# omerbt/TokenFlow

Hardware: NVIDIA H100
Metric: frames/sec for 40-frame 512x512 SD1.5 50-step edit (higher is better)
Workload: dtype fp16

## Files before the change

include/tokenflow_b200.h:

```cpp
#ifndef TOKENFLOW_B200_H_
#define TOKENFLOW_B200_H_

#include <stdint.h>

#ifdef __cplusplus
extern "C" {
#endif

typedef void* tf_stream_t;

#define TF_MAX_FRAMES 64
#define TF_MAX_ATTN_SAMPLES 160

int tf_version(void);
const char* tf_last_error(void);
int64_t tf_launch_count(void);

int tf_unit_rows(const void* x, int x_is_f32, int64_t rows, int dim, int64_t x_row_stride, void* out_f16,
                 tf_stream_t stream);

int tf_layernorm_unit_rows(const void* x_f16, int64_t rows, int dim, int64_t x_row_stride, const float* gamma,
                           const float* beta, float eps, void* out_f16, tf_stream_t stream);

int tf_layernorm_rows(const void* x_f16, int64_t rows, int dim, int64_t x_row_stride, const float* gamma,
// ... 15 lines not shown
                         const int32_t* q_slab, const int32_t* k_slab0, const int32_t* v_slab0,
                         const int32_t* n_kv, int S, int heads, int d, float scale, int q_row0, int q_nrows,
                         void* out, tf_stream_t stream);

int tf_cfg_ddim(const void* eps_uncond, const void* eps_cond, const void* x, const float* coef, float guidance,
                int64_t n, void* out, tf_stream_t stream);

int tf_ddim(const void* eps, const void* x, const float* coef, int64_t n, void* out, tf_stream_t stream);


int tf_cfg_ddim_v(const void* v_uncond, const void* v_cond, const void* x, const float* coef, float guidance,
                  int64_t n, void* out, tf_stream_t stream);

int tf_ddim_v(const void* v, const void* x, const float* coef, int64_t n, void* out, tf_stream_t stream);


int64_t tf_group_norm_nhwc_workspace(int64_t n, int64_t hw, int c, int groups);
int tf_group_norm_nhwc(const void* x, const void* bias, int64_t bias_stride, const void* gamma, const void* beta,
                       int64_t n, int64_t hw, int c, int groups, float eps, int silu, void* workspace,
                       int64_t workspace_bytes, void* out, tf_stream_t stream);

int tf_geglu(const void* xh, const void* gate, int64_t n, void* out, tf_stream_t stream);


int tf_frames_to_nhwc(const void* frames_u8, int64_t n_px, void* out_f16, tf_stream_t stream);

int tf_nhwc_to_frames(const void* x_f16, int64_t n_px, void* frames_u8, tf_stream_t stream);

int tf_resize_taps(int in, int out);
int tf_resize_coeffs(int in, int out, int32_t* bounds, int32_t* coeffs);
int tf_resize_u8(const void* in, int64_t n, int h_in, int w_in, int h, int w, const int32_t* h_bounds,
                 const int32_t* h_coeffs, int h_taps, const int32_t* v_bounds, const int32_t* v_coeffs, int v_taps,
                 void* tmp, void* out, tf_stream_t stream);

int64_t tf_canny_workspace(int64_t n, int h, int w);
int tf_canny_u8(const void* frames, int64_t n, int h, int w, double low, double high, void* workspace,
                int64_t workspace_bytes, void* edges_u8, void* cond_f16, tf_stream_t stream);

#define TF_COMM_ID_BYTES 128
typedef void* tf_comm_t;
int tf_comm_nccl_version(void);
int tf_comm_unique_id(void* id_out);
int tf_comm_init(const void* id, int nranks, int rank, tf_comm_t* comm_out);
int tf_allgather(tf_comm_t comm, const void* send, void* recv, int64_t bytes_per_rank, tf_stream_t stream);
int tf_comm_destroy(tf_comm_t comm);

// ... 5 lines not shown
```

tokenflow_b200/_build.py:

```python
from __future__ import annotations

import hashlib
import os
import shutil
import subprocess
import sys
from pathlib import Path

PKG_DIR = Path(__file__).resolve().parent
CSRC = PKG_DIR / "csrc"
LIB_PATH = PKG_DIR / "libtokenflow_b200.so"
STAMP = PKG_DIR / ".libtokenflow_b200.stamp"

SOURCES = ["tf_capi.cu", "tf_unit_rows.cu", "tf_propagate.cu", "tf_nn_field.cu", "tf_ext_attn.cu", "tf_cfg_ddim.cu",
           "tf_comm.cu", "tf_body.cu", "tf_pixels.cu", "tf_resize.cu",
           "tf_canny.cu"]
HEADERS = ["tf_common.cuh", "tf_kernels.h", "tf_wgmma.cuh", "../../include/tokenflow_b200.h"]

NVCC_FLAGS = [
    "-gencode", "arch=compute_90a,code=sm_90a",
    "-O3", "-std=c++17", "-lineinfo",
    "-Xcompiler", "-fPIC",
    "-Xcompiler", "-ffp-contract=off",
    "-Xptxas", "-v",
    "--expt-relaxed-constexpr",
    "-cudart", "static",
]


def _nvcc() -> str:
    for cand in (os.environ.get("NVCC"), shutil.which("nvcc"), "/usr/local/cuda/bin/nvcc"):
        if cand and os.path.exists(cand):
            return cand
    raise RuntimeError("nvcc not found (set NVCC=/path/to/nvcc)")


def _digest() -> str:
    h = hashlib.sha256()
    for name in SOURCES + HEADERS:
        h.update((CSRC / name).read_bytes())
# ... 43 lines not shown
```

tokenflow_b200/csrc/tf_body.cu:

```cuda
#include "tf_common.cuh"
#include "tf_kernels.h"

namespace tf {
namespace {

constexpr int kGnMaxThreads = 512;
static_assert(kGnMaxChannels / 8 <= kGnMaxThreads, "one row of 8-channel columns must fit in a CTA");
constexpr int kGnStatsChunkBytes = 64 << 10;
constexpr int kGnApplyChunkBytes = 128 << 10;
constexpr int kGnUnroll = 4;

struct GnLayout {
  int cols, rows, threads;
  long long stats_px, apply_px;
  int stats_chunks, apply_chunks;
};

GnLayout gn_layout(long long hw, int c) {
  GnLayout L;
  L.cols = c / 8;
  L.rows = kGnMaxThreads / L.cols > 0 ? kGnMaxThreads / L.cols : 1;
  L.threads = (L.cols * L.rows + 31) / 32 * 32;
  auto chunk = [&](int bytes) {
    long long px = bytes / (2LL * c);
// ... 191 lines not shown
      if (q < p_end) {
        float v[8];
        unpack8(raw[u], v);
        uint4 w;
        __half2* h = reinterpret_cast<__half2*>(&w);
#pragma unroll
        for (int e = 0; e < 4; ++e) {
          float y[2];
#pragma unroll
          for (int k = 0; k < 2; ++k) {
            const int i = 2 * e + k;
            const float xv = kBias ? round_h(v[i] + bv[i]) : v[i];
            y[k] = round_h(fmaf(a[i], xv, b[i]));
            if (kSilu) y[k] = y[k] / (1.0f + expf(-y[k]));
          }
          h[e] = __floats2half2_rn(y[0], y[1]);
        }
        *reinterpret_cast<uint4*>(on + q * C + c0) = w;
      }
    }
  }
}

__device__ __forceinline__ float gelu_erf(float v) {
  constexpr float kAlpha = 0.70710678118654752440f;
  return v * 0.5f * (1.0f + erff(v * kAlpha));
}

__device__ __forceinline__ float geglu1(float xv, float gv) { return xv * round_h(gelu_erf(gv)); }

__global__ void __launch_bounds__(256)
geglu_kernel(const __half* __restrict__ xh, const __half* __restrict__ gate, long long n_vec, long long n,
             __half* __restrict__ out) {
  const long long stride = (long long)gridDim.x * blockDim.x;
  for (long long i = (long long)blockIdx.x * blockDim.x + threadIdx.x; i < n_vec; i += stride) {
    float xv[8], gv[8];
    unpack8(reinterpret_cast<const uint4*>(xh)[i], xv);
    unpack8(reinterpret_cast<const uint4*>(gate)[i], gv);
    uint4 w;
    __half2* h = reinterpret_cast<__half2*>(&w);
#pragma unroll
    for (int e = 0; e < 4; ++e) h[e] = __floats2half2_rn(geglu1(xv[2 * e], gv[2 * e]), geglu1(xv[2 * e + 1], gv[2 * e + 1]));
    reinterpret_cast<uint4*>(out)[i] = w;
  }
  if (blockIdx.x == 0 && threadIdx.x == 0) {
    for (long long j = n_vec * 8; j < n; ++j)
      out[j] = __float2half_rn(geglu1(__half2float(xh[j]), __half2float(gate[j])));
  }
}

}

long long group_norm_nhwc_workspace(long long n, long long hw, int c, int groups) {
  if (n <= 0 || hw <= 0 || c <= 0 || (c & 7) || groups <= 0 || c % groups) return 0;
  return n * groups * (long long)gn_layout(hw, c).stats_chunks * (long long)sizeof(double2);
}

namespace {

template <int kCpg>
int launch_gn(const GnLayout& L, const __half* xp, const __half* bp, long long bias_stride, const __half* gp,
              const __half* btp, long long n, long long hw, int c, int groups, float eps, int silu, double2* ws,
              __half* op, cudaStream_t stream, const char* stats_what, const char* apply_what) {
  const int cpg = c / groups;
  const size_t stats_smem = (size_t)L.threads * 2 * sizeof(double2);
  const size_t apply_smem = (2 * (size_t)c + 2 * (size_t)groups) * sizeof(float);
  for (long long n0 = 0; n0 < n; n0 += 65535) {
    const unsigned ny = (unsigned)(n - n0 < 65535 ? n - n0 : 65535);
    const long long off = n0 * hw * c;
    const __half* bn = bp ? bp + n0 * bias_stride : nullptr;
// ... 60 lines not shown
```

tokenflow_b200/csrc/tf_capi.cu:

```cuda
#include <algorithm>
#include <atomic>
#include <cmath>
#include <cstdarg>
#include <cstdio>
#include <cstring>
#include <initializer_list>
#include <vector>

#include "../../include/tokenflow_b200.h"
#include "tf_common.cuh"
#include "tf_kernels.h"

namespace tf {

static thread_local char g_err[512] = "";
static std::atomic<long long> g_launches{0};

void set_last_error(const char* fmt, ...) {
  va_list ap;
  va_start(ap, fmt);
  vsnprintf(g_err, sizeof(g_err), fmt, ap);
  va_end(ap);
}

// ... 335 lines not shown
  if (!canny_sizes_ok(n, h, w, "tf_canny_u8")) return TF_ERR_INVALID_ARGUMENT;
  if (!(low == low) || !(high == high)) {
    set_last_error("tf_canny_u8: NaN threshold");
    return TF_ERR_INVALID_ARGUMENT;
  }
  if (low > high) std::swap(low, high);
  const double lo = std::floor(low), hi = std::floor(high);
  const int ilo = (int)std::min(std::max(lo, -1.0), 2040.0), ihi = (int)std::min(std::max(hi, -1.0), 2040.0);
  if (n == 0) return TF_OK;
  const long long need = canny_workspace(n, h, w);
  if (workspace_bytes < need) {
    set_last_error("tf_canny_u8: workspace of %lld bytes, %lld needed", (long long)workspace_bytes, need);
    return TF_ERR_INVALID_ARGUMENT;
  }
  const bool cond_ok = !(reinterpret_cast<uintptr_t>(cond_f16) & 1u);
  if (int e = check_pointers("tf_canny_u8", {workspace}, {}, frames && (edges_u8 || cond_f16) && cond_ok)) return e;
  return launched(
      launch_canny(frames, n, h, w, ilo, ihi, workspace, edges_u8, cond_f16, static_cast<cudaStream_t>(stream)), 5);
}

int tf_geglu(const void* xh, const void* gate, int64_t n, void* out, tf_stream_t stream) {
  return elementwise("tf_geglu", n, INT64_MAX, {xh, gate, out}, true,
                     [&] { return launch_geglu(xh, gate, n, out, static_cast<cudaStream_t>(stream)); });
}

int tf_nn_field(const void* x_unit, const void* piv_unit, const int32_t* kf_a, const int32_t* kf_b, int F, int S,
                int dim, int K, int32_t* idx_a, int32_t* idx_b, tf_stream_t stream) {
  if (F < 0 || S < 0 || dim <= 0 || (dim & 7) || K <= 0) {
    set_last_error("tf_nn_field: bad shape F=%d S=%d dim=%d K=%d", F, S, dim, K);
    return TF_ERR_INVALID_ARGUMENT;
  }
  std::vector<FrameChunk> chunks;
  bool need_b;
  if (int e = frame_chunks(chunks, need_b, kf_a, kf_b, nullptr, F, K, "tf_nn_field")) return e;
  if (F == 0 || S == 0) return TF_OK;
  if (int e = check_pointers("tf_nn_field", {x_unit, piv_unit}, {}, idx_a && (!need_b || idx_b))) return e;
  const __half* xu = static_cast<const __half*>(x_unit);
  for (const FrameChunk& c : chunks) {
    const long long off = (long long)c.f0 * S;
    if (int e = launched(launch_nn_field(xu + off * dim, piv_unit, c.tab, c.n, S, dim, K, idx_a + off,
                                         idx_b ? idx_b + off : nullptr, static_cast<cudaStream_t>(stream))))
      return e;
  }
  return TF_OK;
}

// ... 144 lines not shown
```

tokenflow_b200/csrc/tf_common.cuh:

```cuda
#pragma once

#include <cuda.h>
#include <cuda_fp16.h>
#include <cuda_runtime.h>
#include <stdint.h>
#include <stdio.h>

namespace tf {

void set_last_error(const char* fmt, ...);
int  check_cuda(cudaError_t e, const char* what);

enum Status : int {
  TF_OK = 0,
  TF_ERR_INVALID_ARGUMENT = 1,
  TF_ERR_CUDA = 2,
  TF_ERR_UNSUPPORTED = 3,
  TF_ERR_DRIVER = 4,
};

CUresult encode_tiled(CUtensorMap* map, CUtensorMapDataType dtype, uint32_t rank, const void* base,
                      const uint64_t* dims, const uint64_t* strides_bytes ,
                      const uint32_t* box, CUtensorMapSwizzle swizzle);

// ... 29 lines not shown
      : "memory");
  return ok != 0;
}
__device__ __forceinline__ uint64_t global_timer_ns() {
  uint64_t t;
  asm volatile("mov.u64 %0, %%globaltimer;" : "=l"(t));
  return t;
}
__device__ __forceinline__ void mbar_wait(uint64_t* bar, uint32_t parity) {
  uint32_t spins = 0;
  uint64_t t0 = 0;
  while (!mbar_try_wait(bar, parity)) {
    if ((++spins & 2047u) == 0) {
      const uint64_t now = global_timer_ns();
      if (t0 == 0) t0 = now;
      if (now - t0 > 2000000000ull) __trap();
    }
  }
}

__device__ __forceinline__ void tma_prefetch_desc(const CUtensorMap* m) {
  asm volatile("prefetch.tensormap [%0];" ::"l"(reinterpret_cast<uint64_t>(m)) : "memory");
}
__device__ __forceinline__ void tma_load_3d(void* smem_dst, const CUtensorMap* m, uint64_t* bar, int c0,
                                            int c1, int c2) {
  asm volatile(
      "cp.async.bulk.tensor.3d.shared::cluster.global.tile.mbarrier::complete_tx::bytes"
      " [%0], [%1, {%3, %4, %5}], [%2];"
      ::"r"(smem_u32(smem_dst)), "l"(reinterpret_cast<uint64_t>(m)), "r"(smem_u32(bar)), "r"(c0), "r"(c1),
      "r"(c2)
      : "memory");
}
__device__ __forceinline__ void tma_load_4d(void* smem_dst, const CUtensorMap* m, uint64_t* bar, int c0,
                                            int c1, int c2, int c3) {
  asm volatile(
      "cp.async.bulk.tensor.4d.shared::cluster.global.tile.mbarrier::complete_tx::bytes"
      " [%0], [%1, {%3, %4, %5, %6}], [%2];"
      ::"r"(smem_u32(smem_dst)), "l"(reinterpret_cast<uint64_t>(m)), "r"(smem_u32(bar)), "r"(c0), "r"(c1),
      "r"(c2), "r"(c3)
      : "memory");
}

__device__ __forceinline__ uint64_t wgmma_desc(uint32_t smem_addr, uint32_t lbo_bytes, uint32_t sbo_bytes) {
  uint64_t d = 0;
  d |= static_cast<uint64_t>((smem_addr & 0x3FFFFu) >> 4);
  d |= static_cast<uint64_t>((lbo_bytes >> 4) & 0x3FFFu) << 16;
  d |= static_cast<uint64_t>((sbo_bytes >> 4) & 0x3FFFu) << 32;
  d |= static_cast<uint64_t>(1) << 62;
  return d;
}
__device__ __forceinline__ void wgmma_fence() { asm volatile("wgmma.fence.sync.aligned;" ::: "memory"); }
__device__ __forceinline__ void wgmma_commit() { asm volatile("wgmma.commit_group.sync.aligned;" ::: "memory"); }
template <int kPending>
__device__ __forceinline__ void wgmma_wait() {
  asm volatile("wgmma.wait_group.sync.aligned %0;" ::"n"(kPending) : "memory");
}
template <int N>
__device__ __forceinline__ void reg_fence(float (&r)[N]) {
#pragma unroll
  for (int i = 0; i < N; ++i) asm volatile("" : "+f"(r[i])::"memory");
}

__device__ __forceinline__ uint32_t pack_f16x2_rn(float lo, float hi) {
  uint32_t r;
  asm("cvt.rn.f16x2.f32 %0, %1, %2;" : "=r"(r) : "f"(hi), "f"(lo));
  return r;
}
__device__ __forceinline__ float fast_exp2(float x) {
  float y;
  asm("ex2.approx.ftz.f32 %0, %1;" : "=f"(y) : "f"(x));
  return y;
}
#endif

}
```

tokenflow_b200/csrc/tf_kernels.h:

```cpp
#pragma once

#include <cuda_runtime.h>
#include <stdint.h>

namespace tf {

constexpr int kMaxFrames = 64;
struct FrameTable {
  int32_t kf_a[kMaxFrames];
  int32_t kf_b[kMaxFrames];
  float w[kMaxFrames];
};

int launch_unit_rows(const void* x, int x_is_f32, long long rows, int dim, long long row_stride, void* out_f16,
                     cudaStream_t stream);

int launch_layernorm_unit_rows(const void* x_f16, long long rows, int dim, long long row_stride, const float* gamma,
                               const float* beta, float eps, void* out_f16, cudaStream_t stream);

int launch_layernorm_rows(const void* x_f16, long long rows, int dim, long long row_stride, const float* gamma,
                          const float* beta, float eps, void* y_out, long long y_row_stride, void* unit_out,
                          long long unit_row_stride, long long unit_rows, cudaStream_t stream);

int launch_cfg_ddim(const void* eps_uncond, const void* eps_cond, const void* x, const float* coef_dev, float guidance,
                    long long n, void* out, cudaStream_t stream);
int launch_ddim(const void* eps, const void* x, const float* coef_dev, long long n, void* out, cudaStream_t stream);
int launch_cfg_ddim_v(const void* v_uncond, const void* v_cond, const void* x, const float* coef_dev, float guidance,
                      long long n, void* out, cudaStream_t stream);
int launch_ddim_v(const void* v, const void* x, const float* coef_dev, long long n, void* out, cudaStream_t stream);

constexpr int kGnMaxChannels = 4096;
long long group_norm_nhwc_workspace(long long n, long long hw, int c, int groups);
int launch_group_norm_nhwc(const void* x, const void* bias, long long bias_stride, const void* gamma, const void* beta,
                           long long n, long long hw, int c, int groups, float eps, int silu, void* workspace,
                           void* out, cudaStream_t stream);
int launch_geglu(const void* xh, const void* gate, long long n, void* out, cudaStream_t stream);

int launch_frames_to_nhwc(const void* frames, long long n, void* out, cudaStream_t stream);
int launch_nhwc_to_frames(const void* x, long long n, void* frames, cudaStream_t stream);

int resize_taps(int in, int out);
void resize_coeffs(int in, int out, int32_t* bounds, int32_t* coeffs);
int launch_resize_h(const void* in, long long n_rows, int w_in, int w, const int32_t* bounds, const int32_t* coeffs,
                    int taps, void* out, cudaStream_t stream);
int launch_resize_v(const void* in, long long n, int h_in, int h, int w, const int32_t* bounds, const int32_t* coeffs,
                    int taps, void* out, cudaStream_t stream);

long long canny_workspace(long long n, int h, int w);
int launch_canny(const void* frames, long long n, int h, int w, int low, int high, void* workspace, void* edges,
                 void* cond, cudaStream_t stream);

int launch_propagate(const void* A, const int32_t* idx_a, const int32_t* idx_b, const FrameTable& tab, int F,
                     int S, int dim, int K, const void* residual, void* out, int out_is_f32, long long F_total,
                     cudaStream_t stream);

int launch_nn_field(const void* x_unit, const void* piv_unit, const FrameTable& tab, int F, int S, int dim,
                    int K, int32_t* idx_a, int32_t* idx_b, cudaStream_t stream);

struct AttnSample {
// ... 35 lines not shown
```

tokenflow_b200/csrc/tf_wgmma.cuh:

```cuda
#pragma once

#include <stdint.h>

namespace tf {

template <int N> __device__ __forceinline__ void wgmma_ss(float (&d)[N / 2], uint64_t a, uint64_t b, uint32_t acc);
template <int N> __device__ __forceinline__ void wgmma_rs(float (&d)[N / 2], const uint32_t (&a)[4], uint64_t b, uint32_t acc);

template <>
__device__ __forceinline__ void wgmma_ss<64>(float (&d)[32], uint64_t a, uint64_t b, uint32_t acc) {
  asm volatile(
      "{\n\t.reg .pred p;\n\t"
      "setp.ne.b32 p, %34, 0;\n\t"
      "wgmma.mma_async.sync.aligned.m64n64k16.f32.f16.f16 "
      "{%0, %1, %2, %3, %4, %5, %6, %7, %8, %9, %10, %11, %12, %13, %14, %15, %16, %17, %18, %19, %20, %21, %22, %23, %24, %25, %26, %27, %28, %29, %30, %31}, "
      "%32, %33, p, 1, 1, 0, 0;\n\t}\n"
      : "+f"(d[0]), "+f"(d[1]), "+f"(d[2]), "+f"(d[3]), "+f"(d[4]), "+f"(d[5]), "+f"(d[6]), "+f"(d[7]),
        "+f"(d[8]), "+f"(d[9]), "+f"(d[10]), "+f"(d[11]), "+f"(d[12]), "+f"(d[13]), "+f"(d[14]), "+f"(d[15]),
        "+f"(d[16]), "+f"(d[17]), "+f"(d[18]), "+f"(d[19]), "+f"(d[20]), "+f"(d[21]), "+f"(d[22]), "+f"(d[23]),
        "+f"(d[24]), "+f"(d[25]), "+f"(d[26]), "+f"(d[27]), "+f"(d[28]), "+f"(d[29]), "+f"(d[30]), "+f"(d[31])
      : "l"(a), "l"(b), "r"(acc));
}

template <>
__device__ __forceinline__ void wgmma_ss<128>(float (&d)[64], uint64_t a, uint64_t b, uint32_t acc) {
  asm volatile(
      "{\n\t.reg .pred p;\n\t"
      "setp.ne.b32 p, %66, 0;\n\t"
      "wgmma.mma_async.sync.aligned.m64n128k16.f32.f16.f16 "
      "{%0, %1, %2, %3, %4, %5, %6, %7, %8, %9, %10, %11, %12, %13, %14, %15, %16, %17, %18, %19, %20, %21, %22, %23, %24, %25, %26, %27, %28, %29, %30, %31, %32, %33, %34, %35, %36, %37, %38, %39, %40, %41, %42, %43, %44, %45, %46, %47, %48, %49, %50, %51, %52, %53, %54, %55, %56, %57, %58, %59, %60, %61, %62, %63}, "
// ... 199 lines not shown
template <>
__device__ __forceinline__ void wgmma_rs<192>(float (&d)[96], const uint32_t (&a)[4], uint64_t b, uint32_t acc) {
  asm volatile(
      "{\n\t.reg .pred p;\n\t"
      "setp.ne.b32 p, %101, 0;\n\t"
      "wgmma.mma_async.sync.aligned.m64n192k16.f32.f16.f16 "
      "{%0, %1, %2, %3, %4, %5, %6, %7, %8, %9, %10, %11, %12, %13, %14, %15, %16, %17, %18, %19, %20, %21, %22, %23, %24, %25, %26, %27, %28, %29, %30, %31, %32, %33, %34, %35, %36, %37, %38, %39, %40, %41, %42, %43, %44, %45, %46, %47, %48, %49, %50, %51, %52, %53, %54, %55, %56, %57, %58, %59, %60, %61, %62, %63, %64, %65, %66, %67, %68, %69, %70, %71, %72, %73, %74, %75, %76, %77, %78, %79, %80, %81, %82, %83, %84, %85, %86, %87, %88, %89, %90, %91, %92, %93, %94, %95}, "
      "{%96, %97, %98, %99}, %100, p, 1, 1, 1;\n\t}\n"
      : "+f"(d[0]), "+f"(d[1]), "+f"(d[2]), "+f"(d[3]), "+f"(d[4]), "+f"(d[5]), "+f"(d[6]), "+f"(d[7]),
        "+f"(d[8]), "+f"(d[9]), "+f"(d[10]), "+f"(d[11]), "+f"(d[12]), "+f"(d[13]), "+f"(d[14]), "+f"(d[15]),
        "+f"(d[16]), "+f"(d[17]), "+f"(d[18]), "+f"(d[19]), "+f"(d[20]), "+f"(d[21]), "+f"(d[22]), "+f"(d[23]),
        "+f"(d[24]), "+f"(d[25]), "+f"(d[26]), "+f"(d[27]), "+f"(d[28]), "+f"(d[29]), "+f"(d[30]), "+f"(d[31]),
        "+f"(d[32]), "+f"(d[33]), "+f"(d[34]), "+f"(d[35]), "+f"(d[36]), "+f"(d[37]), "+f"(d[38]), "+f"(d[39]),
        "+f"(d[40]), "+f"(d[41]), "+f"(d[42]), "+f"(d[43]), "+f"(d[44]), "+f"(d[45]), "+f"(d[46]), "+f"(d[47]),
        "+f"(d[48]), "+f"(d[49]), "+f"(d[50]), "+f"(d[51]), "+f"(d[52]), "+f"(d[53]), "+f"(d[54]), "+f"(d[55]),
        "+f"(d[56]), "+f"(d[57]), "+f"(d[58]), "+f"(d[59]), "+f"(d[60]), "+f"(d[61]), "+f"(d[62]), "+f"(d[63]),
        "+f"(d[64]), "+f"(d[65]), "+f"(d[66]), "+f"(d[67]), "+f"(d[68]), "+f"(d[69]), "+f"(d[70]), "+f"(d[71]),
        "+f"(d[72]), "+f"(d[73]), "+f"(d[74]), "+f"(d[75]), "+f"(d[76]), "+f"(d[77]), "+f"(d[78]), "+f"(d[79]),
        "+f"(d[80]), "+f"(d[81]), "+f"(d[82]), "+f"(d[83]), "+f"(d[84]), "+f"(d[85]), "+f"(d[86]), "+f"(d[87]),
        "+f"(d[88]), "+f"(d[89]), "+f"(d[90]), "+f"(d[91]), "+f"(d[92]), "+f"(d[93]), "+f"(d[94]), "+f"(d[95])
      : "r"(a[0]), "r"(a[1]), "r"(a[2]), "r"(a[3]), "l"(b), "r"(acc));
}

}
```

tokenflow_b200/ops.py:

```python
from __future__ import annotations

import ctypes
import math
from pathlib import Path
from typing import Optional, Sequence, Tuple

import torch

LIB_NAME = "libtokenflow_b200.so"
TF_MAX_FRAMES = 64
TF_MAX_ATTN_SAMPLES = 160
TF_COMM_ID_BYTES = 128

_c_i32p = ctypes.POINTER(ctypes.c_int32)
_c_f32p = ctypes.POINTER(ctypes.c_float)

_SIGNATURES = {
    "tf_version": (ctypes.c_int, []),
    "tf_last_error": (ctypes.c_char_p, []),
    "tf_launch_count": (ctypes.c_int64, []),
    "tf_unit_rows": (ctypes.c_int, [ctypes.c_void_p, ctypes.c_int, ctypes.c_int64, ctypes.c_int, ctypes.c_int64,
                                    ctypes.c_void_p, ctypes.c_void_p]),
    "tf_layernorm_unit_rows": (ctypes.c_int, [ctypes.c_void_p, ctypes.c_int64, ctypes.c_int, ctypes.c_int64,
                                              ctypes.c_void_p, ctypes.c_void_p, ctypes.c_float, ctypes.c_void_p,
                                              ctypes.c_void_p]),
    "tf_layernorm_rows": (ctypes.c_int, [ctypes.c_void_p, ctypes.c_int64, ctypes.c_int, ctypes.c_int64, ctypes.c_void_p,
                                         ctypes.c_void_p, ctypes.c_float, ctypes.c_void_p, ctypes.c_int64,
                                         ctypes.c_void_p, ctypes.c_int64, ctypes.c_int64, ctypes.c_void_p]),
    "tf_cfg_ddim": (ctypes.c_int, [ctypes.c_void_p, ctypes.c_void_p, ctypes.c_void_p, ctypes.c_void_p, ctypes.c_float,
                                   ctypes.c_int64, ctypes.c_void_p, ctypes.c_void_p]),
    "tf_ddim": (ctypes.c_int, [ctypes.c_void_p, ctypes.c_void_p, ctypes.c_void_p, ctypes.c_int64, ctypes.c_void_p,
                               ctypes.c_void_p]),
    "tf_cfg_ddim_v": (ctypes.c_int, [ctypes.c_void_p, ctypes.c_void_p, ctypes.c_void_p, ctypes.c_void_p,
                                     ctypes.c_float, ctypes.c_int64, ctypes.c_void_p, ctypes.c_void_p]),
    "tf_ddim_v": (ctypes.c_int, [ctypes.c_void_p, ctypes.c_void_p, ctypes.c_void_p, ctypes.c_int64, ctypes.c_void_p,
                                 ctypes.c_void_p]),
    "tf_comm_nccl_version": (ctypes.c_int, []),
    "tf_comm_unique_id": (ctypes.c_int, [ctypes.c_void_p]),
# ... 10 lines not shown
                                       ctypes.c_int, ctypes.c_void_p, ctypes.c_void_p]),
    "tf_ext_attn_fwd_rows": (ctypes.c_int, [ctypes.c_void_p, ctypes.c_int, ctypes.c_int64, ctypes.c_void_p,
                                            ctypes.c_void_p, ctypes.c_int, ctypes.c_int64, ctypes.c_int, _c_i32p,
                                            _c_i32p, _c_i32p, _c_i32p, _c_i32p, ctypes.c_int, ctypes.c_int,
                                            ctypes.c_int, ctypes.c_float, ctypes.c_int, ctypes.c_int, ctypes.c_void_p,
                                            ctypes.c_void_p]),
    "tf_group_norm_nhwc_workspace": (ctypes.c_int64, [ctypes.c_int64, ctypes.c_int64, ctypes.c_int, ctypes.c_int]),
    "tf_group_norm_nhwc": (ctypes.c_int, [ctypes.c_void_p, ctypes.c_void_p, ctypes.c_int64, ctypes.c_void_p,
                                          ctypes.c_void_p, ctypes.c_int64, ctypes.c_int64, ctypes.c_int, ctypes.c_int,
                                          ctypes.c_float, ctypes.c_int, ctypes.c_void_p, ctypes.c_int64,
                                          ctypes.c_void_p, ctypes.c_void_p]),
    "tf_frames_to_nhwc": (ctypes.c_int, [ctypes.c_void_p, ctypes.c_int64, ctypes.c_void_p, ctypes.c_void_p]),
    "tf_nhwc_to_frames": (ctypes.c_int, [ctypes.c_void_p, ctypes.c_int64, ctypes.c_void_p, ctypes.c_void_p]),
    "tf_resize_taps": (ctypes.c_int, [ctypes.c_int, ctypes.c_int]),
    "tf_resize_coeffs": (ctypes.c_int, [ctypes.c_int, ctypes.c_int, ctypes.c_void_p, ctypes.c_void_p]),
    "tf_resize_u8": (ctypes.c_int, [ctypes.c_void_p, ctypes.c_int64, ctypes.c_int, ctypes.c_int, ctypes.c_int,
                                    ctypes.c_int, ctypes.c_void_p, ctypes.c_void_p, ctypes.c_int, ctypes.c_void_p,
                                    ctypes.c_void_p, ctypes.c_int, ctypes.c_void_p, ctypes.c_void_p, ctypes.c_void_p]),
    "tf_canny_workspace": (ctypes.c_int64, [ctypes.c_int64, ctypes.c_int, ctypes.c_int]),
    "tf_canny_u8": (ctypes.c_int, [ctypes.c_void_p, ctypes.c_int64, ctypes.c_int, ctypes.c_int, ctypes.c_double,
                                   ctypes.c_double, ctypes.c_void_p, ctypes.c_int64, ctypes.c_void_p, ctypes.c_void_p,
                                   ctypes.c_void_p]),
    "tf_geglu": (ctypes.c_int, [ctypes.c_void_p, ctypes.c_void_p, ctypes.c_int64, ctypes.c_void_p, ctypes.c_void_p]),
}


class TokenflowB200Error(RuntimeError):
    pass


def library_path() -> Path:
    return Path(__file__).resolve().parent / LIB_NAME


_LIB = None


def load_library() -> ctypes.CDLL:
    global _LIB
    if _LIB is not None:
        return _LIB
    path = library_path()
    if not path.exists():
        raise TokenflowB200Error(
            f"{path} is missing: build it with `python -m tokenflow_b200._build` "
            "(or __graft_entry__.build()).  tokenflow_b200 has no fallback path.")
# ... 68 lines not shown
    def __init__(self):
        self.lib = load_library()
        if not torch.cuda.is_available():
            raise TokenflowB200Error(
                "tokenflow_b200 needs a CUDA device (sm_90a / H100); there is no CPU path.")
        major, minor = torch.cuda.get_device_capability()
        if (major, minor) != (9, 0):
            raise TokenflowB200Error(f"tokenflow_b200 kernels are compiled for sm_90a only (got sm_{major}{minor})")

    @staticmethod
    def _stream() -> int:
        return torch.cuda.current_stream().cuda_stream

    def launch_count(self) -> int:
        return int(self.lib.tf_launch_count())

    _timing = None

    def enable_timing(self, on: bool = True):
        self._timing = [] if on else None

    def _launch(self, timer: str, work: float, fn: str, *args):
        entry = getattr(self.lib, fn)
        if self._timing is None:
            return _check(self.lib, entry(*args, self._stream()), fn)
        ext = torch.cuda.is_current_stream_capturing()
        start = torch.cuda.Event(enable_timing=True, external=ext)
        end = torch.cuda.Event(enable_timing=True, external=ext)
        start.record()
        _check(self.lib, entry(*args, self._stream()), fn)
        end.record()
        self._timing.append((timer, float(work), start, end))

    def timing_summary(self):
        torch.cuda.synchronize()
        agg = {}
        for name, work, s, e in (self._timing or []):
            a = agg.setdefault(name, {"launches": 0, "ms": 0.0, "work": 0.0})
            a["launches"] += 1
            a["ms"] += s.elapsed_time(e)
            a["work"] += work
        if self._timing is not None:
            self._timing = []
        return agg

    def unit_rows(self, x: torch.Tensor) -> torch.Tensor:
        if x.dtype not in (torch.float32, torch.float16):
            x = x.float()
        dim = x.shape[-1]
        x2 = _rows(x.reshape(-1, dim), 4)
        out = torch.empty(x2.shape, dtype=torch.float16, device=x.device)
        nbytes = x2.shape[0] * dim * (x2.element_size() + 2)
        self._launch("tf_unit_rows", nbytes, "tf_unit_rows", x2.data_ptr(), int(x2.dtype == torch.float32), x2.shape[0],
# ... 258 lines not shown
        ws = torch.empty(max(ws_bytes, 16), dtype=torch.uint8, device=dev)
        e = c = None
        if edges:
            e = out_edges if out_edges is not None else torch.empty((n, h, w), dtype=torch.uint8, device=dev)
            assert e.shape == (n, h, w) and e.dtype == torch.uint8 and e.is_contiguous()
        if cond:
            c = out_cond if out_cond is not None else torch.empty((n, 3, h, w), dtype=torch.float16, device=dev,
                                                                  memory_format=torch.channels_last)
            assert c.shape == (n, 3, h, w) and c.dtype == torch.float16 and c.is_contiguous(memory_format=torch.channels_last)
        work = 3.0 * n * h * w + (n * h * w if edges else 0) + (6.0 * n * h * w if cond else 0)
        ptr = lambda t: t.data_ptr() if t is not None else None
        self._launch("tf_canny_u8", work, "tf_canny_u8", frames.data_ptr(), n, h, w, float(low), float(high),
                     ws.data_ptr(), ws.numel(), ptr(e), ptr(c))
        return e, c

    def geglu(self, xh: torch.Tensor, gate: torch.Tensor) -> torch.Tensor:
        assert xh.dtype == gate.dtype == torch.float16 and xh.shape == gate.shape
        xh, gate = _dense(xh), _dense(gate)
        out = torch.empty_like(xh)
        n = xh.numel()
        self._launch("tf_geglu", 3.0 * n * 2, "tf_geglu", xh.data_ptr(), gate.data_ptr(), n, out.data_ptr())
        return out


_DEFAULT_OPS = None


def default_ops() -> CudaOps:
    global _DEFAULT_OPS
    if _DEFAULT_OPS is None:
        _DEFAULT_OPS = CudaOps()
    return _DEFAULT_OPS


_BODY_OPS = False


def body_ops() -> Optional[CudaOps]:
    global _BODY_OPS
    if _BODY_OPS is False:
        try:
            _BODY_OPS = default_ops()
        except TokenflowB200Error:
            _BODY_OPS = None
    return _BODY_OPS

# ... 61 lines not shown
```

tokenflow_b200/sd_unet.py:

```python
from __future__ import annotations

import math
from dataclasses import dataclass
from typing import Optional, Tuple

import torch
import torch.nn as nn
import torch.nn.functional as F


@dataclass
class UNetConfig:
    in_channels: int = 4
    out_channels: int = 4
    block_out_channels: Tuple[int, ...] = (320, 640, 1280, 1280)
    layers_per_block: int = 2
    cross_attention_dim: int = 768
    num_heads: Tuple[int, ...] = (8, 8, 8, 8)
    norm_num_groups: int = 32
    use_linear_projection: bool = False
    sample_size: Optional[int] = 64


_ENCODER_FIXED = {
# ... 140 lines not shown

class GEGLU(nn.Module):
    def __init__(self, dim_in: int, dim_out: int):
        super().__init__()
        self.proj = nn.Linear(dim_in, dim_out * 2)

    def forward(self, x):
        w_x, w_g = self.proj.weight.chunk(2, dim=0)
        b_x, b_g = self.proj.bias.chunk(2, dim=0)
        xh, g = F.linear(x, w_x, b_x), F.linear(x, w_g, b_g)
        if xh.is_cuda and xh.dtype == g.dtype == torch.float16:
            from .ops import body_ops
            ops = body_ops()
            if ops is not None:
                return ops.geglu(xh, g)
        return xh * F.gelu(g)


class FeedForward(nn.Module):
    def __init__(self, dim: int, mult: int = 4):
        super().__init__()
        self.net = nn.ModuleList([GEGLU(dim, dim * mult), nn.Dropout(0.0), nn.Linear(dim * mult, dim)])

    def forward(self, x):
        for m in self.net:
            x = m(x)
        return x


class BasicTransformerBlock(nn.Module):

    def __init__(self, dim: int, heads: int, dim_head: int, cross_attention_dim: int):
        super().__init__()
        self.only_cross_attention = False
        self.use_ada_layer_norm = False
        self.use_ada_layer_norm_zero = False
        self.norm1 = nn.LayerNorm(dim)
        self.attn1 = Attention(dim, None, heads, dim_head)
        self.norm2 = BodyLayerNorm(dim)
        self.attn2 = Attention(dim, cross_attention_dim, heads, dim_head)
        self.norm3 = BodyLayerNorm(dim)
        self.ff = FeedForward(dim)

    def forward(self, hidden_states, attention_mask=None, encoder_hidden_states=None,
                encoder_attention_mask=None, timestep=None, cross_attention_kwargs=None,
                class_labels=None):
        hidden_states = self.attn1(self.norm1(hidden_states)) + hidden_states
        hidden_states = self.attn2(self.norm2(hidden_states),
                                   encoder_hidden_states=encoder_hidden_states,
                                   attention_mask=encoder_attention_mask) + hidden_states
        return self.ff(self.norm3(hidden_states)) + hidden_states


class Transformer2DModel(nn.Module):
    def __init__(self, channels: int, heads: int, cross_attention_dim: int, groups: int, linear_proj: bool):
        super().__init__()
        self.use_linear_projection = linear_proj
        self.norm = GroupNorm(groups, channels, eps=1e-6)
        if linear_proj:
            self.proj_in = nn.Linear(channels, channels)
            self.proj_out = nn.Linear(channels, channels)
        else:
            self.proj_in = nn.Conv2d(channels, channels, 1)
            self.proj_out = nn.Conv2d(channels, channels, 1)
        self.transformer_blocks = nn.ModuleList(
            [BasicTransformerBlock(channels, heads, channels // heads, cross_attention_dim)])

    def forward(self, hidden_states, encoder_hidden_states=None):
        b, c, hh, ww = hidden_states.shape
        residual = hidden_states
        x = norm_act(self.norm, hidden_states, silu=False)
        if self.use_linear_projection:
            x = x.permute(0, 2, 3, 1).reshape(b, hh * ww, c)
            x = self.proj_in(x)
# ... 271 lines not shown
```

tokenflow_b200/tokenflow_utils.py:

```python
from __future__ import annotations

import os
import weakref
from typing import List, Optional, Sequence, Type

import torch

from . import ops as tf_ops
from .sd_unet import norm_act
from .util import isinstance_str, batch_cosine_sim

__all__ = [
    "register_pivotal", "register_batch_idx", "register_frame_table", "register_shard", "register_fused",
    "PivotalShard", "set_strict_dtype",
    "register_time", "load_source_latents_t",
    "register_conv_injection", "register_extended_attention_pnp", "register_extended_attention",
    "make_tokenflow_attention_block", "set_tokenflow", "isinstance_str", "batch_cosine_sim",
]

_OPS = None


def _ops():
    global _OPS
# ... 339 lines not shown
                    encoder_attention_mask=None, timestep=None, cross_attention_kwargs=None,
                    class_labels=None) -> torch.Tensor:
            if getattr(self, "use_ada_layer_norm", False) or getattr(self, "use_ada_layer_norm_zero", False):
                raise NotImplementedError(
                    "tokenflow_b200: AdaLayerNorm transformer blocks are not part of any Stable-Diffusion "
                    "UNet and are not supported by the H100 hot path")
            cross_attention_kwargs = cross_attention_kwargs if cross_attention_kwargs is not None else {}
            n_piv = getattr(self, "_tf_fused", 0)
            if n_piv:
                piv = self._tf_pivotal(hidden_states[:n_piv],
                                       None if encoder_hidden_states is None else encoder_hidden_states[:n_piv],
                                       cross_attention_kwargs)
                frm = self._tf_frames(hidden_states[n_piv:])
                hidden_states = torch.cat([piv, frm.to(piv.dtype) if frm.dtype != piv.dtype else frm])
            elif self.pivotal_pass:
                hidden_states = self._tf_pivotal(hidden_states, encoder_hidden_states, cross_attention_kwargs)
            else:
                hidden_states = self._tf_frames(hidden_states)

            if self.attn2 is not None:
                attn_output = self.attn2(self.norm2(hidden_states), encoder_hidden_states=encoder_hidden_states,
                                         attention_mask=encoder_attention_mask, **cross_attention_kwargs)
                hidden_states = attn_output + hidden_states
            return self.ff(self.norm3(hidden_states)) + hidden_states

        def _tf_pivotal(self, hidden_states, encoder_hidden_states, cross_attention_kwargs):
            ops = _ops()
            batch_size, sequence_length, dim = hidden_states.shape
            shard = getattr(self, "_tf_shard", None)
            fused_ln = (hidden_states.is_cuda and hidden_states.dtype == torch.float16
                        and hasattr(ops, "layernorm_rows") and not self.only_cross_attention
                        and (torch.is_autocast_enabled() or self.norm1.weight.dtype == torch.float16))
            n_unit = batch_size if shard is not None else batch_size // 3
            if fused_ln:
                norm_hidden_states, unit = ops.layernorm_rows(hidden_states, self.norm1, n_unit)
            else:
                norm_hidden_states = self.norm1(hidden_states)
                unit = ops.unit_rows(norm_hidden_states[:n_unit])
            if shard is not None:
                self.attn1._tf_unit_local = unit
                self.pivot_hidden_states = norm_hidden_states
                self.attn_output = self.attn1(norm_hidden_states, **cross_attention_kwargs)
                unit_all = self.attn1.__dict__.pop("_tf_unit_gathered", None)
                full = self.attn1.__dict__.pop("_tf_attn_full", None)
                if unit_all is None or full is None:
                    raise RuntimeError("tokenflow_b200: a sharded pivotal pass needs the extended-attention attn1 of "
                                       "register_extended_attention[_pnp]; this block's attn1 did not gather the pivot "
# ... 52 lines not shown
```

Baseline: 2.913.

## Fuse GEGLU activation, down-projection GEMM, bias and residual into one WGMMA kernel

Adds a TMA-fed, three-stage pipelined WGMMA kernel that loads the GEGLU x and gate halves, applies GELU in registers, and feeds the result as the register A operand of the down-projection. Bias and the residual add happen in the epilogue. This removes the separate geglu kernel, the round trip of the 4n-wide intermediate through global memory, and a separate residual add. The up-projection is split into two F.linear calls, which may cost more than a single GEMM plus chunk. Only widths 320 and 640 use the fused path; 1280 falls back to the old code.

```diff
diff --git a/include/tokenflow_b200.h b/include/tokenflow_b200.h
--- a/include/tokenflow_b200.h
+++ b/include/tokenflow_b200.h
@@ -61,6 +61,19 @@
 
 int tf_geglu(const void* xh, const void* gate, int64_t n, void* out, tf_stream_t stream);
 
+typedef struct {
+  const void* xh;
+  const void* gate;
+  const void* w;
+  const void* bias;
+  const void* residual;
+  void* out;
+  int64_t m;
+  int n;
+  tf_stream_t stream;
+} tf_ff_call;
+int tf_ff_down_geglu(const tf_ff_call* call);
+
 
 int tf_frames_to_nhwc(const void* frames_u8, int64_t n_px, void* out_f16, tf_stream_t stream);
 
diff --git a/tokenflow_b200/_build.py b/tokenflow_b200/_build.py
--- a/tokenflow_b200/_build.py
+++ b/tokenflow_b200/_build.py
@@ -14,8 +14,8 @@
 
 SOURCES = ["tf_capi.cu", "tf_unit_rows.cu", "tf_propagate.cu", "tf_nn_field.cu", "tf_ext_attn.cu", "tf_cfg_ddim.cu",
            "tf_comm.cu", "tf_body.cu", "tf_pixels.cu", "tf_resize.cu",
-           "tf_canny.cu"]
-HEADERS = ["tf_common.cuh", "tf_kernels.h", "tf_wgmma.cuh", "../../include/tokenflow_b200.h"]
+           "tf_canny.cu", "tf_ff.cu"]
+HEADERS = ["tf_common.cuh", "tf_geglu.cuh", "tf_kernels.h", "tf_wgmma.cuh", "../../include/tokenflow_b200.h"]
 
 NVCC_FLAGS = [
     "-gencode", "arch=compute_90a,code=sm_90a",
diff --git a/tokenflow_b200/csrc/tf_body.cu b/tokenflow_b200/csrc/tf_body.cu
--- a/tokenflow_b200/csrc/tf_body.cu
+++ b/tokenflow_b200/csrc/tf_body.cu
@@ -1,4 +1,5 @@
 #include "tf_common.cuh"
+#include "tf_geglu.cuh"
 #include "tf_kernels.h"
 
 namespace tf {
@@ -237,30 +238,22 @@
   }
 }
 
-__device__ __forceinline__ float gelu_erf(float v) {
-  constexpr float kAlpha = 0.70710678118654752440f;
-  return v * 0.5f * (1.0f + erff(v * kAlpha));
-}
-
-__device__ __forceinline__ float geglu1(float xv, float gv) { return xv * round_h(gelu_erf(gv)); }
-
 __global__ void __launch_bounds__(256)
 geglu_kernel(const __half* __restrict__ xh, const __half* __restrict__ gate, long long n_vec, long long n,
              __half* __restrict__ out) {
   const long long stride = (long long)gridDim.x * blockDim.x;
   for (long long i = (long long)blockIdx.x * blockDim.x + threadIdx.x; i < n_vec; i += stride) {
-    float xv[8], gv[8];
-    unpack8(reinterpret_cast<const uint4*>(xh)[i], xv);
-    unpack8(reinterpret_cast<const uint4*>(gate)[i], gv);
+    const uint4 xv = reinterpret_cast<const uint4*>(xh)[i], gv = reinterpret_cast<const uint4*>(gate)[i];
+    const __half2* x2 = reinterpret_cast<const __half2*>(&xv);
+    const __half2* g2 = reinterpret_cast<const __half2*>(&gv);
     uint4 w;
     __half2* h = reinterpret_cast<__half2*>(&w);
 #pragma unroll
-    for (int e = 0; e < 4; ++e) h[e] = __floats2half2_rn(geglu1(xv[2 * e], gv[2 * e]), geglu1(xv[2 * e + 1], gv[2 * e + 1]));
+    for (int e = 0; e < 4; ++e) h[e] = geglu2(x2[e], g2[e]);
     reinterpret_cast<uint4*>(out)[i] = w;
   }
   if (blockIdx.x == 0 && threadIdx.x == 0) {
-    for (long long j = n_vec * 8; j < n; ++j)
-      out[j] = __float2half_rn(geglu1(__half2float(xh[j]), __half2float(gate[j])));
+    for (long long j = n_vec * 8; j < n; ++j) out[j] = __low2half(geglu2(__half2half2(xh[j]), __half2half2(gate[j])));
   }
 }
 
diff --git a/tokenflow_b200/csrc/tf_capi.cu b/tokenflow_b200/csrc/tf_capi.cu
--- a/tokenflow_b200/csrc/tf_capi.cu
+++ b/tokenflow_b200/csrc/tf_capi.cu
@@ -381,6 +381,23 @@
 int tf_geglu(const void* xh, const void* gate, int64_t n, void* out, tf_stream_t stream) {
   return elementwise("tf_geglu", n, INT64_MAX, {xh, gate, out}, true,
                      [&] { return launch_geglu(xh, gate, n, out, static_cast<cudaStream_t>(stream)); });
+}
+
+int tf_ff_down_geglu(const tf_ff_call* call) {
+  if (!call) { set_last_error("tf_ff_down_geglu: NULL call"); return TF_ERR_INVALID_ARGUMENT; }
+  const tf_ff_call& c = *call;
+  if (c.m < 0 || c.m > INT32_MAX - 127 || c.n <= 0) {
+    set_last_error("tf_ff_down_geglu: bad shape m=%lld n=%d", (long long)c.m, c.n);
+    return TF_ERR_INVALID_ARGUMENT;
+  }
+  if (!ff_down_geglu_supported(c.n)) {
+    set_last_error("tf_ff_down_geglu: n=%d not supported (320, 640 or 1280)", c.n);
+    return TF_ERR_UNSUPPORTED;
+  }
+  if (c.m == 0) return TF_OK;
+  if (int e = check_pointers("tf_ff_down_geglu", {c.xh, c.gate, c.w, c.bias, c.residual, c.out})) return e;
+  return launched(launch_ff_down_geglu(c.xh, c.gate, c.w, c.bias, c.residual, c.m, c.n, c.out,
+                                       static_cast<cudaStream_t>(c.stream)));
 }
 
 int tf_nn_field(const void* x_unit, const void* piv_unit, const int32_t* kf_a, const int32_t* kf_b, int F, int S,
diff --git a/tokenflow_b200/csrc/tf_common.cuh b/tokenflow_b200/csrc/tf_common.cuh
--- a/tokenflow_b200/csrc/tf_common.cuh
+++ b/tokenflow_b200/csrc/tf_common.cuh
@@ -75,6 +75,13 @@
 __device__ __forceinline__ void tma_prefetch_desc(const CUtensorMap* m) {
   asm volatile("prefetch.tensormap [%0];" ::"l"(reinterpret_cast<uint64_t>(m)) : "memory");
 }
+__device__ __forceinline__ void tma_load_2d(void* smem_dst, const CUtensorMap* m, uint64_t* bar, int c0, int c1) {
+  asm volatile(
+      "cp.async.bulk.tensor.2d.shared::cluster.global.tile.mbarrier::complete_tx::bytes"
+      " [%0], [%1, {%3, %4}], [%2];"
+      ::"r"(smem_u32(smem_dst)), "l"(reinterpret_cast<uint64_t>(m)), "r"(smem_u32(bar)), "r"(c0), "r"(c1)
+      : "memory");
+}
 __device__ __forceinline__ void tma_load_3d(void* smem_dst, const CUtensorMap* m, uint64_t* bar, int c0,
                                             int c1, int c2) {
   asm volatile(
@@ -114,6 +121,13 @@
   for (int i = 0; i < N; ++i) asm volatile("" : "+f"(r[i])::"memory");
 }
 
+__device__ __forceinline__ void ldmatrix_x4(uint32_t (&r)[4], uint32_t smem_addr) {
+  asm volatile("ldmatrix.sync.aligned.m8n8.x4.shared.b16 {%0, %1, %2, %3}, [%4];"
+               : "=r"(r[0]), "=r"(r[1]), "=r"(r[2]), "=r"(r[3])
+               : "r"(smem_addr)
+               : "memory");
+}
+
 __device__ __forceinline__ uint32_t pack_f16x2_rn(float lo, float hi) {
   uint32_t r;
   asm("cvt.rn.f16x2.f32 %0, %1, %2;" : "=r"(r) : "f"(hi), "f"(lo));
diff --git a/tokenflow_b200/csrc/tf_ff.cu b/tokenflow_b200/csrc/tf_ff.cu
--- /dev/null
+++ b/tokenflow_b200/csrc/tf_ff.cu
@@ -0,0 +1,172 @@
+#include "tf_common.cuh"
+#include "tf_geglu.cuh"
+#include "tf_kernels.h"
+#include "tf_wgmma.cuh"
+
+namespace tf {
+namespace {
+
+constexpr int kBlockM = 128;
+constexpr int kBlockN = 320;
+constexpr int kHalfN = kBlockN / 2;
+constexpr int kChunkK = 64;
+constexpr int kStages = 3;
+constexpr int kXBytes = kBlockM * 128;
+constexpr int kWHalfBytes = kHalfN * 128;
+constexpr int kStageBytes = 2 * kXBytes + 2 * kWHalfBytes;
+constexpr int kThreads = 256;
+
+struct FfCtl {
+  uint64_t full[kStages];
+  uint64_t empty[kStages];
+};
+
+__device__ __forceinline__ uint32_t geglu_pack(uint32_t x2, uint32_t g2) {
+  const __half2 a = geglu2(*reinterpret_cast<const __half2*>(&x2), *reinterpret_cast<const __half2*>(&g2));
+  return *reinterpret_cast<const uint32_t*>(&a);
+}
+
+__device__ __forceinline__ float round_h(float x) { return __half2float(__float2half_rn(x)); }
+
+__global__ void __launch_bounds__(kThreads, 1)
+ff_down_geglu_kernel(const __grid_constant__ CUtensorMap map_x, const __grid_constant__ CUtensorMap map_g,
+                     const __grid_constant__ CUtensorMap map_w, const __half* __restrict__ bias,
+                     const __half* __restrict__ residual, long long M, int N, int n_tiles, int k_chunks,
+                     __half* __restrict__ out) {
+  extern __shared__ uint8_t smem_raw[];
+  uint8_t* smem = reinterpret_cast<uint8_t*>((reinterpret_cast<uintptr_t>(smem_raw) + 1023) & ~uintptr_t(1023));
+  FfCtl* ctl = reinterpret_cast<FfCtl*>(smem + kStages * kStageBytes);
+  const int nt = blockIdx.x % n_tiles;
+  const int m0 = (blockIdx.x / n_tiles) * kBlockM;
+  const int n0 = nt * kBlockN;
+
+  if (threadIdx.x == 0) {
+    tma_prefetch_desc(&map_x);
+    tma_prefetch_desc(&map_g);
+    tma_prefetch_desc(&map_w);
+    for (int i = 0; i < kStages; ++i) {
+      mbar_init(&ctl->full[i], 1);
+      mbar_init(&ctl->empty[i], 8);
+    }
+    fence_mbar_init();
+  }
+  __syncthreads();
+
+  auto load = [&](int j) {
+    const int st = j % kStages;
+    uint8_t* dst = smem + st * kStageBytes;
+    mbar_arrive_expect_tx(&ctl->full[st], (uint32_t)kStageBytes);
+    tma_load_2d(dst, &map_x, &ctl->full[st], j * kChunkK, m0);
+    tma_load_2d(dst + kXBytes, &map_g, &ctl->full[st], j * kChunkK, m0);
+    tma_load_2d(dst + 2 * kXBytes, &map_w, &ctl->full[st], j * kChunkK, n0);
+    tma_load_2d(dst + 2 * kXBytes + kWHalfBytes, &map_w, &ctl->full[st], j * kChunkK, n0 + kHalfN);
+  };
+  if (threadIdx.x == 0)
+    for (int j = 0; j < kStages && j < k_chunks; ++j) load(j);
+
+  const int wg = threadIdx.x >> 7;
+  const int warp = (threadIdx.x >> 5) & 3;
+  const int lane = threadIdx.x & 31;
+  const int lrow = wg * 64 + warp * 16 + (lane & 15);
+  const uint32_t row_addr = smem_u32(smem) + lrow * 128;
+  const int swz = lrow & 7;
+  const int khalf = lane >> 4;
+
+  float acc[2][kHalfN / 2];
+  uint32_t a[kChunkK / 16][4];
+  for (int j = 0; j < k_chunks; ++j) {
+    const int st = j % kStages;
+    mbar_wait(&ctl->full[st], (uint32_t)(j / kStages) & 1u);
+    __syncwarp();
+    const uint32_t stage = (uint32_t)(st * kStageBytes);
+    const uint32_t w_addr = smem_u32(smem) + stage + 2 * kXBytes;
+#pragma unroll
+    for (int kk = 0; kk < kChunkK / 16; ++kk) {
+      wgmma_wait<3>();
+      if (kk == kChunkK / 16 - 1 && j > 0) {
+        const int ps = (j - 1) % kStages;
+        __syncwarp();
+        if (lane == 0) mbar_arrive(&ctl->empty[ps]);
+        if (threadIdx.x == 0 && j - 1 + kStages < k_chunks) {
+          mbar_wait(&ctl->empty[ps], (uint32_t)((j - 1) / kStages) & 1u);
+          load(j - 1 + kStages);
+        }
+        __syncwarp();
+      }
+      const uint32_t chunk = (uint32_t)(((2 * kk + khalf) ^ swz) << 4);
+      uint32_t xr[4], gr[4];
+      ldmatrix_x4(xr, row_addr + stage + chunk);
+      ldmatrix_x4(gr, row_addr + stage + kXBytes + chunk);
+#pragma unroll
+      for (int e = 0; e < 4; ++e) a[kk][e] = geglu_pack(xr[e], gr[e]);
+      const uint32_t accum = (j > 0 || kk > 0) ? 1u : 0u;
+      wgmma_fence();
+      wgmma_rs_kb<kHalfN>(acc[0], a[kk], wgmma_desc(w_addr + kk * 32, 16, 1024), accum);
+      wgmma_rs_kb<kHalfN>(acc[1], a[kk], wgmma_desc(w_addr + kWHalfBytes + kk * 32, 16, 1024), accum);
+      wgmma_commit();
+    }
+  }
+  wgmma_wait<0>();
+  reg_fence(acc[0]);
+  reg_fence(acc[1]);
+
+  const long long row = m0 + wg * 64 + warp * 16 + (lane >> 2);
+  const int qcol = 2 * (lane & 3);
+#pragma unroll
+  for (int h = 0; h < 2; ++h) {
+#pragma unroll
+    for (int jb = 0; jb < kHalfN / 8; ++jb) {
+      const int c = n0 + h * kHalfN + 8 * jb + qcol;
+      const float2 bv = __half22float2(*reinterpret_cast<const __half2*>(bias + c));
+#pragma unroll
+      for (int r = 0; r < 2; ++r) {
+        const long long m = row + 8 * r;
+        if (m < M) {
+          const float2 rv = __half22float2(*reinterpret_cast<const __half2*>(residual + m * N + c));
+          const float y0 = round_h(acc[h][4 * jb + 2 * r] + bv.x) + rv.x;
+          const float y1 = round_h(acc[h][4 * jb + 2 * r + 1] + bv.y) + rv.y;
+          *reinterpret_cast<uint32_t*>(out + m * N + c) = pack_f16x2_rn(y0, y1);
+        }
+      }
+    }
+  }
+}
+
+}
+
+bool ff_down_geglu_supported(int n) { return n == 320 || n == 640 || n == 1280; }
+
+int launch_ff_down_geglu(const void* xh, const void* gate, const void* w, const void* bias, const void* residual,
+                         long long m, int n, void* out, cudaStream_t stream) {
+  if (m == 0) return TF_OK;
+  const int k = 4 * n;
+  CUtensorMap map_x, map_g, map_w;
+  auto make = [&](CUtensorMap* map, const void* base, long long rows, int box_rows, const char* what) -> int {
+    const uint64_t dims[2] = {(uint64_t)k, (uint64_t)rows};
+    const uint64_t strides[1] = {(uint64_t)k * 2};
+    const uint32_t box[2] = {(uint32_t)kChunkK, (uint32_t)box_rows};
+    CUresult r = encode_tiled(map, CU_TENSOR_MAP_DATA_TYPE_FLOAT16, 2, base, dims, strides, box,
+                              CU_TENSOR_MAP_SWIZZLE_128B);
+    if (r != CUDA_SUCCESS) {
+      set_last_error("tf_ff_down_geglu: cuTensorMapEncodeTiled(%s) failed: %d", what, (int)r);
+      return TF_ERR_DRIVER;
+    }
+    return TF_OK;
+  };
+  if (int e = make(&map_x, xh, m, kBlockM, "xh")) return e;
+  if (int e = make(&map_g, gate, m, kBlockM, "gate")) return e;
+  if (int e = make(&map_w, w, n, kHalfN, "w")) return e;
+  const size_t smem_bytes = 1024 + (size_t)kStages * kStageBytes + sizeof(FfCtl);
+  if (check_cuda(cudaFuncSetAttribute(ff_down_geglu_kernel, cudaFuncAttributeMaxDynamicSharedMemorySize,
+                                      (int)smem_bytes),
+                 "tf_ff_down_geglu smem attribute"))
+    return TF_ERR_CUDA;
+  const int n_tiles = n / kBlockN;
+  const long long grid = (m + kBlockM - 1) / kBlockM * n_tiles;
+  ff_down_geglu_kernel<<<(unsigned)grid, kThreads, smem_bytes, stream>>>(
+      map_x, map_g, map_w, static_cast<const __half*>(bias), static_cast<const __half*>(residual), m, n, n_tiles,
+      k / kChunkK, static_cast<__half*>(out));
+  return check_cuda(cudaGetLastError(), "tf_ff_down_geglu launch");
+}
+
+}
diff --git a/tokenflow_b200/csrc/tf_geglu.cuh b/tokenflow_b200/csrc/tf_geglu.cuh
--- /dev/null
+++ b/tokenflow_b200/csrc/tf_geglu.cuh
@@ -0,0 +1,17 @@
+#pragma once
+
+#include <cuda_fp16.h>
+
+namespace tf {
+
+__device__ __forceinline__ float gelu_erf(float v) {
+  constexpr float kAlpha = 0.70710678118654752440f;
+  return v * 0.5f * (1.0f + erff(v * kAlpha));
+}
+
+__device__ __forceinline__ __half2 geglu2(__half2 xh, __half2 g) {
+  const float2 gf = __half22float2(g);
+  return __hmul2(xh, __floats2half2_rn(gelu_erf(gf.x), gelu_erf(gf.y)));
+}
+
+}
diff --git a/tokenflow_b200/csrc/tf_kernels.h b/tokenflow_b200/csrc/tf_kernels.h
--- a/tokenflow_b200/csrc/tf_kernels.h
+++ b/tokenflow_b200/csrc/tf_kernels.h
@@ -35,6 +35,9 @@
                            long long n, long long hw, int c, int groups, float eps, int silu, void* workspace,
                            void* out, cudaStream_t stream);
 int launch_geglu(const void* xh, const void* gate, long long n, void* out, cudaStream_t stream);
+bool ff_down_geglu_supported(int n);
+int launch_ff_down_geglu(const void* xh, const void* gate, const void* w, const void* bias, const void* residual,
+                         long long m, int n, void* out, cudaStream_t stream);
 
 int launch_frames_to_nhwc(const void* frames, long long n, void* out, cudaStream_t stream);
 int launch_nhwc_to_frames(const void* x, long long n, void* frames, cudaStream_t stream);
diff --git a/tokenflow_b200/csrc/tf_wgmma.cuh b/tokenflow_b200/csrc/tf_wgmma.cuh
--- a/tokenflow_b200/csrc/tf_wgmma.cuh
+++ b/tokenflow_b200/csrc/tf_wgmma.cuh
@@ -6,6 +6,7 @@
 
 template <int N> __device__ __forceinline__ void wgmma_ss(float (&d)[N / 2], uint64_t a, uint64_t b, uint32_t acc);
 template <int N> __device__ __forceinline__ void wgmma_rs(float (&d)[N / 2], const uint32_t (&a)[4], uint64_t b, uint32_t acc);
+template <int N> __device__ __forceinline__ void wgmma_rs_kb(float (&d)[N / 2], const uint32_t (&a)[4], uint64_t b, uint32_t acc);
 
 template <>
 __device__ __forceinline__ void wgmma_ss<64>(float (&d)[32], uint64_t a, uint64_t b, uint32_t acc) {
@@ -251,4 +252,25 @@
       : "r"(a[0]), "r"(a[1]), "r"(a[2]), "r"(a[3]), "l"(b), "r"(acc));
 }
 
-}
+template <>
+__device__ __forceinline__ void wgmma_rs_kb<160>(float (&d)[80], const uint32_t (&a)[4], uint64_t b, uint32_t acc) {
+  asm volatile(
+      "{\n\t.reg .pred p;\n\t"
+      "setp.ne.b32 p, %85, 0;\n\t"
+      "wgmma.mma_async.sync.aligned.m64n160k16.f32.f16.f16 "
+      "{%0, %1, %2, %3, %4, %5, %6, %7, %8, %9, %10, %11, %12, %13, %14, %15, %16, %17, %18, %19, %20, %21, %22, %23, %24, %25, %26, %27, %28, %29, %30, %31, %32, %33, %34, %35, %36, %37, %38, %39, %40, %41, %42, %43, %44, %45, %46, %47, %48, %49, %50, %51, %52, %53, %54, %55, %56, %57, %58, %59, %60, %61, %62, %63, %64, %65, %66, %67, %68, %69, %70, %71, %72, %73, %74, %75, %76, %77, %78, %79}, "
+      "{%80, %81, %82, %83}, %84, p, 1, 1, 0;\n\t}\n"
+      : "+f"(d[0]), "+f"(d[1]), "+f"(d[2]), "+f"(d[3]), "+f"(d[4]), "+f"(d[5]), "+f"(d[6]), "+f"(d[7]),
+        "+f"(d[8]), "+f"(d[9]), "+f"(d[10]), "+f"(d[11]), "+f"(d[12]), "+f"(d[13]), "+f"(d[14]), "+f"(d[15]),
+        "+f"(d[16]), "+f"(d[17]), "+f"(d[18]), "+f"(d[19]), "+f"(d[20]), "+f"(d[21]), "+f"(d[22]), "+f"(d[23]),
+        "+f"(d[24]), "+f"(d[25]), "+f"(d[26]), "+f"(d[27]), "+f"(d[28]), "+f"(d[29]), "+f"(d[30]), "+f"(d[31]),
+        "+f"(d[32]), "+f"(d[33]), "+f"(d[34]), "+f"(d[35]), "+f"(d[36]), "+f"(d[37]), "+f"(d[38]), "+f"(d[39]),
+        "+f"(d[40]), "+f"(d[41]), "+f"(d[42]), "+f"(d[43]), "+f"(d[44]), "+f"(d[45]), "+f"(d[46]), "+f"(d[47]),
+        "+f"(d[48]), "+f"(d[49]), "+f"(d[50]), "+f"(d[51]), "+f"(d[52]), "+f"(d[53]), "+f"(d[54]), "+f"(d[55]),
+        "+f"(d[56]), "+f"(d[57]), "+f"(d[58]), "+f"(d[59]), "+f"(d[60]), "+f"(d[61]), "+f"(d[62]), "+f"(d[63]),
+        "+f"(d[64]), "+f"(d[65]), "+f"(d[66]), "+f"(d[67]), "+f"(d[68]), "+f"(d[69]), "+f"(d[70]), "+f"(d[71]),
+        "+f"(d[72]), "+f"(d[73]), "+f"(d[74]), "+f"(d[75]), "+f"(d[76]), "+f"(d[77]), "+f"(d[78]), "+f"(d[79])
+      : "r"(a[0]), "r"(a[1]), "r"(a[2]), "r"(a[3]), "l"(b), "r"(acc));
+}
+
+}
diff --git a/tokenflow_b200/ops.py b/tokenflow_b200/ops.py
--- a/tokenflow_b200/ops.py
+++ b/tokenflow_b200/ops.py
@@ -14,6 +14,13 @@
 
 _c_i32p = ctypes.POINTER(ctypes.c_int32)
 _c_f32p = ctypes.POINTER(ctypes.c_float)
+
+
+
+class FfCall(ctypes.Structure):
+    _fields_ = [(name, ctypes.c_void_p) for name in ("xh", "gate", "w", "bias", "residual", "out")] + [
+        ("m", ctypes.c_int64), ("n", ctypes.c_int), ("stream", ctypes.c_void_p)]
+
 
 _SIGNATURES = {
     "tf_version": (ctypes.c_int, []),
@@ -70,6 +77,7 @@
                                    ctypes.c_double, ctypes.c_void_p, ctypes.c_int64, ctypes.c_void_p, ctypes.c_void_p,
                                    ctypes.c_void_p]),
     "tf_geglu": (ctypes.c_int, [ctypes.c_void_p, ctypes.c_void_p, ctypes.c_int64, ctypes.c_void_p, ctypes.c_void_p]),
+    "tf_ff_down_geglu": (ctypes.c_int, [ctypes.POINTER(FfCall)]),
 }
 
 
@@ -184,13 +192,15 @@
 
     def _launch(self, timer: str, work: float, fn: str, *args):
         entry = getattr(self.lib, fn)
+        stream_arg = len(args) < len(entry.argtypes)
+        call = (lambda: entry(*args, self._stream())) if stream_arg else (lambda: entry(*args))
         if self._timing is None:
-            return _check(self.lib, entry(*args, self._stream()), fn)
+            return _check(self.lib, call(), fn)
         ext = torch.cuda.is_current_stream_capturing()
         start = torch.cuda.Event(enable_timing=True, external=ext)
         end = torch.cuda.Event(enable_timing=True, external=ext)
         start.record()
-        _check(self.lib, entry(*args, self._stream()), fn)
+        _check(self.lib, call(), fn)
         end.record()
         self._timing.append((timer, float(work), start, end))
 
@@ -495,6 +505,32 @@
         self._launch("tf_geglu", 3.0 * n * 2, "tf_geglu", xh.data_ptr(), gate.data_ptr(), n, out.data_ptr())
         return out
 
+    FF_DOWN_WIDTHS = (320, 640)
+
+    @classmethod
+    def ff_down_geglu_supported(cls, x: torch.Tensor, up: torch.nn.Linear, down: torch.nn.Linear,
+                                residual: torch.Tensor) -> bool:
+        n = x.shape[-1]
+        params = (up.weight, up.bias, down.weight, down.bias)
+        return (n in cls.FF_DOWN_WIDTHS and x.is_cuda and up.bias is not None and down.bias is not None
+                and all(p.dtype == torch.float16 for p in params) and x.dtype == residual.dtype == torch.float16
+                and tuple(up.weight.shape) == (8 * n, n) and tuple(down.weight.shape) == (n, 4 * n)
+                and residual.shape == x.shape and residual.stride(-1) == 1)
+
+    def ff_down_geglu(self, xh: torch.Tensor, g: torch.Tensor, weight: torch.Tensor, bias: torch.Tensor,
+                      residual: torch.Tensor) -> torch.Tensor:
+        n = weight.shape[0]
+        lead = residual.shape[:-1]
+        xh2, g2, r2 = _dense(xh.reshape(-1, 4 * n)), _dense(g.reshape(-1, 4 * n)), _dense(residual.reshape(-1, n))
+        w, b = _dense(weight), _dense(bias)
+        m = r2.shape[0]
+        out = torch.empty((m, n), dtype=torch.float16, device=xh.device)
+        nbytes = 2.0 * m * (2 * 4 * n + 2 * n) + 2.0 * (w.numel() + b.numel())
+        call = FfCall(xh2.data_ptr(), g2.data_ptr(), w.data_ptr(), b.data_ptr(), r2.data_ptr(), out.data_ptr(), m, n,
+                      self._stream())
+        self._launch("tf_geglu", nbytes, "tf_ff_down_geglu", ctypes.byref(call))
+        return out.view(*lead, n)
+
 
 _DEFAULT_OPS = None
 
diff --git a/tokenflow_b200/sd_unet.py b/tokenflow_b200/sd_unet.py
--- a/tokenflow_b200/sd_unet.py
+++ b/tokenflow_b200/sd_unet.py
@@ -186,10 +186,19 @@
         super().__init__()
         self.net = nn.ModuleList([GEGLU(dim, dim * mult), nn.Dropout(0.0), nn.Linear(dim * mult, dim)])
 
-    def forward(self, x):
+    def forward(self, x, residual=None):
+        if residual is not None and x.is_cuda:
+            from .ops import CudaOps, body_ops
+            proj, down = self.net[0].proj, self.net[2]
+            ops = body_ops()
+            if ops is not None and CudaOps.ff_down_geglu_supported(x, proj, down, residual):
+                w_x, w_g = proj.weight.chunk(2, dim=0)
+                b_x, b_g = proj.bias.chunk(2, dim=0)
+                return ops.ff_down_geglu(F.linear(x, w_x, b_x), F.linear(x, w_g, b_g), down.weight, down.bias,
+                                         residual)
         for m in self.net:
             x = m(x)
-        return x
+        return x if residual is None else x + residual
 
 
 class BasicTransformerBlock(nn.Module):
@@ -213,7 +222,7 @@
         hidden_states = self.attn2(self.norm2(hidden_states),
                                    encoder_hidden_states=encoder_hidden_states,
                                    attention_mask=encoder_attention_mask) + hidden_states
-        return self.ff(self.norm3(hidden_states)) + hidden_states
+        return self.ff(self.norm3(hidden_states), residual=hidden_states)
 
 
 class Transformer2DModel(nn.Module):
diff --git a/tokenflow_b200/tokenflow_utils.py b/tokenflow_b200/tokenflow_utils.py
--- a/tokenflow_b200/tokenflow_utils.py
+++ b/tokenflow_b200/tokenflow_utils.py
@@ -385,7 +385,7 @@
                 attn_output = self.attn2(self.norm2(hidden_states), encoder_hidden_states=encoder_hidden_states,
                                          attention_mask=encoder_attention_mask, **cross_attention_kwargs)
                 hidden_states = attn_output + hidden_states
-            return self.ff(self.norm3(hidden_states)) + hidden_states
+            return self.ff(self.norm3(hidden_states), residual=hidden_states)
 
         def _tf_pivotal(self, hidden_states, encoder_hidden_states, cross_attention_kwargs):
             ops = _ops()
```

Result: faster. 2.949, median of 6 (+1.2%).
